# lonewolf-jp/ConvoPeq

Hardware: AMD Instinct MI355X
Metric: Mega stereo-samples/s convolved (131072-tap IR, blk=512) (higher is better)
Workload: dtype f64; 1 GPU; 256 stereo streams per GPU x 1 GPU(s) = 256 streams, 131072-tap IR (private IR per channel), blk 512, fp64 overlap-save conv + 20-band SVF EQ (bench preset, sat 0.2) [BASELINE.json configs[1]]; streams_per_gpu=256, ir_taps=131072, block=512, blocks_per_call=1024, partition=4096, eq=True, eq_preset=bench, parallelism=streams sharded rank-major, 1 rank(s), one per GPU

## Files before the change

### convopeq_amd/csrc/mac_kernels.hip

```cpp
#include "kernels.hpp"

namespace cpq {

namespace {

template <int TT, int PF, int NT = 0>
__global__ __launch_bounds__(256, (TT >= 32 || (TT == 16 && PF >= 16)) ? 1 : 2) void k_fdl_mac(const double2* __restrict__ X, const double2* __restrict__ H,
                                                 const int* __restrict__ irSlot, double2* __restrict__ Y,
                                                 int nPairs, int kPad, int ringMask, int head, int T, int nTiles,
                                                 int64_t hSlotStride, int P, int segShift, int K)
{
    static_assert(TT % PF == 0, "prefetch depth must divide the tile");
    const int bid = blockIdx.x;
    const int xcd = bid & 7;
    const int q = bid >> 3;
    const int tile = q % nTiles;
    const int pair = (q / nTiles) * 8 + xcd;
    if (pair >= nPairs) return;
    const int c = pair >> segShift;
    const int bin = (pair & ((1 << segShift) - 1)) * blockDim.x + threadIdx.x;
    const int t0 = tile * TT;

    const double2* __restrict__ Xc = X + (int64_t)c * (ringMask + 1) * P + bin;
    const double2* __restrict__ Hc = H + (int64_t)irSlot[c] * hSlotStride + bin;
    const int base = head + t0;

    constexpr bool kSplitRe = TT <= 8;
    double2 acc[TT], xw[TT], xn[PF], hn[PF];
    double accq[kSplitRe ? TT : 1];
#pragma unroll
    for (int u = 0; u < TT; ++u) {
        acc[u] = make_double2(0.0, 0.0);
        if (kSplitRe) accq[u] = 0.0;
        xw[u] = Xc[(int64_t)((base + u) & ringMask) * P];
    }
#pragma unroll
    for (int r = 0; r < PF; ++r) {
        xn[r] = Xc[(int64_t)((base - r - 1) & ringMask) * P];
        hn[r] = Hc[(int64_t)r * P];
    }

    for (int k0 = 0; k0 < kPad; k0 += TT) {
#pragma unroll
        for (int r = 0; r < TT; ++r) {
            const int k = k0 + r;
            const double2 h = hn[r % PF];
            const double2 xnew = xn[r % PF];
            if (k + PF < K) {
                if (NT >= 2) {
                    const double* hp = reinterpret_cast<const double*>(Hc + (int64_t)(k + PF) * P);
                    hn[r % PF] = make_double2(__builtin_nontemporal_load(hp), __builtin_nontemporal_load(hp + 1));
                } else {
                    hn[r % PF] = Hc[(int64_t)(k + PF) * P];
                }
            }
            if (k + PF + 1 < K) {
                if (NT >= 1) {
                    const double* xp = reinterpret_cast<const double*>(Xc + (int64_t)((base - (k + PF) - 1) & ringMask) * P);
                    xn[r % PF] = make_double2(__builtin_nontemporal_load(xp), __builtin_nontemporal_load(xp + 1));
                } else {
                    xn[r % PF] = Xc[(int64_t)((base - (k + PF) - 1) & ringMask) * P];
                }
            }
            __builtin_amdgcn_sched_barrier(0);
            if (k < K)
#pragma unroll
            for (int i = 0; i < TT; ++i) {
                const double2 x = xw[(i - r + TT) % TT];
                if (kSplitRe) {
                    acc[i].x = fma(x.x, h.x, acc[i].x);
                    accq[i] = fma(x.y, h.y, accq[i]);
                } else {
                    acc[i].x = fma(x.x, h.x, fma(-x.y, h.y, acc[i].x));
                }
                acc[i].y = fma(x.x, h.y, fma(x.y, h.x, acc[i].y));
            }
            xw[TT - 1 - r] = xnew;
            __builtin_amdgcn_sched_barrier(0);
        }
    }
#pragma unroll
    for (int i = 0; i < TT; ++i)
        if (t0 + i < T) {
            double2 y = acc[i];
            if (kSplitRe) y = (bin == 0) ? make_double2(acc[i].x, accq[i]) : make_double2(acc[i].x - accq[i], acc[i].y);
            Y[((int64_t)c * T + t0 + i) * P + bin] = y;
        }
}

constexpr int kWgWaves = 8;
constexpr int kWgTile = 8;
constexpr int kWgRingBlocks = kWgWaves + 1;
static_assert(kWgWaves == kWgTile, "k_fdl_mac_wg fetches block -1 one row per wave: waves per workgroup == rows per block");

__global__ __launch_bounds__(64 * kWgWaves, 4) void k_fdl_mac_wg(const double2* __restrict__ X,
                                                                  const double2* __restrict__ H,
                                                                  const int* __restrict__ irSlot,
                                                                  double2* __restrict__ Y, int kPad, int ringMask,
                                                                  int head, int T, int nGroups, int64_t hSlotStride,
                                                                  int P, int nCols, int nWork, int K)
{
    __shared__ double2 ring[kWgRingBlocks * kWgTile * 64];
    __shared__ double2 hst[kWgTile * 64];
    const int lane = threadIdx.x & 63;
    const int w = __builtin_amdgcn_readfirstlane(threadIdx.x >> 6);
    const int perXcd = gridDim.x >> 3;
    const int logical = (blockIdx.x & 7) * perXcd + (blockIdx.x >> 3);
    if (logical >= nWork) return;
    const int grp = logical % nGroups;
    const int cg = logical / nGroups;
    const int c = cg / nCols;
    const int bin = (cg - c * nCols) * 64 + lane;
    const int base = head + grp * (kWgWaves * kWgTile);
    const int t0w = grp * (kWgWaves * kWgTile) + w * kWgTile;

    const double2* __restrict__ Xu = X + (int64_t)c * (ringMask + 1) * P;
    const double2* __restrict__ Hu = H + (int64_t)irSlot[c] * hSlotStride;
    auto slotOf = [](int b) { return ((b % kWgRingBlocks) + kWgRingBlocks) % kWgRingBlocks; };
    auto xrow = [&](int slot) { return Xu + (int64_t)(slot & ringMask) * P; };
    auto hrow = [&](int k) { return Hu + (int64_t)k * P; };

    double m1[kWgTile], m2[kWgTile], m3[kWgTile], xsum[kWgTile];
    double2 xw[kWgTile];
#pragma unroll
    for (int u = 0; u < kWgTile; ++u) {
        m1[u] = 0.0; m2[u] = 0.0; m3[u] = 0.0;
        xw[u] = xrow(base + kWgTile * w + u)[bin];
        xsum[u] = xw[u].x + xw[u].y;
    }
    if (w < kWgWaves - 1) {
#pragma unroll
        for (int u = 0; u < kWgTile; ++u) ring[(slotOf(w) * kWgTile + u) * 64 + lane] = xw[u];
    }
    {
        const double2 xs = xrow(base - kWgTile + w)[bin];
        ring[(slotOf(-1) * kWgTile + w) * 64 + lane] = xs;
    }
    hst[w * 64 + lane] = hrow(w)[bin];
    __syncthreads();

    const int nChunks = kPad / kWgTile;
    const int rem = K - (nChunks - 1) * kWgTile;
    const bool active = t0w < T;
    for (int j = 0; j < nChunks; ++j) {
        const bool lastChunk = (j == nChunks - 1), nextIsLast = (j == nChunks - 2);
        const int steps = lastChunk ? rem : kWgTile;
        double2 xs = make_double2(0.0, 0.0), hsn = make_double2(0.0, 0.0);
        if (!lastChunk && (!nextIsLast || w > kWgTile - rem)) {
            const double* xp = reinterpret_cast<const double*>(xrow(base + kWgTile * (-j - 2) + w) + bin);
            xs = make_double2(__builtin_nontemporal_load(xp), __builtin_nontemporal_load(xp + 1));
        }
        if (!lastChunk && (!nextIsLast || w < rem))
            hsn = hrow((j + 1) * kWgTile + w)[bin];
        const double2* blk = ring + slotOf(w - j - 1) * kWgTile * 64 + lane;
        if (active)
#pragma unroll
        for (int r = 0; r < kWgTile; ++r) {
            if (r < steps) {
            const double2 h = hst[r * 64 + lane];
            const double hs = h.x + h.y;
            if (r > 0) xsum[kWgTile - r] = xw[kWgTile - r].x + xw[kWgTile - r].y;
            {
                const double2 x = xw[kWgTile - 1 - r];
                m1[kWgTile - 1] = fma(x.x, h.x, m1[kWgTile - 1]);
                m2[kWgTile - 1] = fma(x.y, h.y, m2[kWgTile - 1]);
                m3[kWgTile - 1] = fma(xsum[kWgTile - 1 - r], hs, m3[kWgTile - 1]);
            }
            xw[kWgTile - 1 - r] = blk[(kWgTile - 1 - r) * 64];
            __builtin_amdgcn_sched_barrier(0);
#pragma unroll
            for (int i = 0; i < kWgTile - 1; ++i) {
                const int sl = (i - r + kWgTile) % kWgTile;
                const double2 x = xw[sl];
                m1[i] = fma(x.x, h.x, m1[i]);
                m2[i] = fma(x.y, h.y, m2[i]);
                m3[i] = fma(xsum[sl], hs, m3[i]);
            }
            __builtin_amdgcn_sched_barrier(0);
            }
        }
        if (lastChunk) break;
        ring[(slotOf(-j - 2) * kWgTile + w) * 64 + lane] = xs;
        xsum[0] = xw[0].x + xw[0].y;
        __syncthreads();
        hst[w * 64 + lane] = hsn;
        __syncthreads();
    }
#pragma unroll
    for (int i = 0; i < kWgTile; ++i)
        if (t0w + i < T) {
            const double2 y = (bin == 0) ? make_double2(m1[i], m2[i]) : make_double2(m1[i] - m2[i], (m3[i] - m1[i]) - m2[i]);
            double* yp = reinterpret_cast<double*>(Y + ((int64_t)c * T + t0w + i) * P + bin);
            __builtin_nontemporal_store(y.x, yp);
            __builtin_nontemporal_store(y.y, yp + 1);
        }
}

__global__ __launch_bounds__(256) void k_fdl_mac_dcnyq(const double2* __restrict__ XDN,
                                                       const double2* __restrict__ HDN,
                                                       const int* __restrict__ irSlot, double2* __restrict__ Y,
                                                       int nCh, int K, int ringMask, int head, int T, int hdnStride, int P)
{
    const int lane = threadIdx.x & 63;
    const int idx = blockIdx.x * (blockDim.x >> 6) + (threadIdx.x >> 6);
    if (idx >= nCh * T) return;
    const int c = idx / T;
    const int t = idx - c * T;
    const double2* __restrict__ x = XDN + (int64_t)c * (ringMask + 1);
    const double2* __restrict__ h = HDN + (int64_t)irSlot[c] * hdnStride;
    double dc = 0.0, ny = 0.0;
    for (int k = lane; k < K; k += 64) {
        const double2 xv = x[(head + t - k) & ringMask];
        const double2 hv = h[k];
        dc = fma(xv.x, hv.x, dc);
        ny = fma(xv.y, hv.y, ny);
    }
#pragma unroll
    for (int off = 32; off > 0; off >>= 1) {
        dc += __shfl_down(dc, off);
        ny += __shfl_down(ny, off);
    }
    if (lane == 0) Y[(int64_t)idx * P] = make_double2(dc, ny);
}

template <int TT, int PF>
void launch_mac_t(hipStream_t stream, const double2* X, const double2* H, const int* irSlot, double2* Y, int P,
                  int nCh, int kPad, int K, int ringSlots, int head, int T, int64_t hSlotStride, bool hPrivate = false)
{
    const int threads = P < 256 ? P : 256;
    int segShift = 0;
    while ((threads << segShift) < P) ++segShift;
    const int nPairs = nCh << segShift;
    const int nTiles = (T + TT - 1) / TT;
    const int groups = (nPairs + 7) / 8;
    const int grid = groups * nTiles * 8;
    if constexpr (TT <= 8) {
        if (nTiles == 1) {
            if (hPrivate)
                hipLaunchKernelGGL((k_fdl_mac<TT, PF, 2>), dim3(grid), dim3(threads), 0, stream, X, H, irSlot, Y, nPairs, kPad,
                                   ringSlots - 1, head, T, nTiles, hSlotStride, P, segShift, K);
            else
                hipLaunchKernelGGL((k_fdl_mac<TT, PF, 1>), dim3(grid), dim3(threads), 0, stream, X, H, irSlot, Y, nPairs, kPad,
                                   ringSlots - 1, head, T, nTiles, hSlotStride, P, segShift, K);
            return;
        }
    }
    hipLaunchKernelGGL((k_fdl_mac<TT, PF>), dim3(grid), dim3(threads), 0, stream, X, H, irSlot, Y, nPairs, kPad,
                       ringSlots - 1, head, T, nTiles, hSlotStride, P, segShift, K);
}

}

int fdl_mac_variant(int tile, int T)
{
    if (tile) return tile;
    if (T >= 48) return 0;
    if (T >= 12) return 16;
    if (T >= 6) return 8;
    return 4;
}

bool fdl_mac_needs_dcnyq(int tile, int T) { return fdl_mac_variant(tile, T) > 8; }

int fdl_mac_kpad_align(int tile, int T)
{
    const int v = fdl_mac_variant(tile, T);
    return v == 0 ? kWgTile : v;
}

void launch_fdl_mac(hipStream_t stream, int tile, const double2* X, const double2* H, const int* irSlot, double2* Y,
                    int P, int nCh, int K, int ringSlots, int head, int T, int64_t hSlotStride, bool hPrivate)
{
    const int kAlign = fdl_mac_kpad_align(tile, T);
    const int kPad = (K + kAlign - 1) / kAlign * kAlign;
    tile = fdl_mac_variant(tile, T);
    if (tile == 0) {
        const int nGroups = (T + kWgWaves * kWgTile - 1) / (kWgWaves * kWgTile);
        const int nCols = P / 64;
        const int nWork = nCh * nCols * nGroups;
        hipLaunchKernelGGL(k_fdl_mac_wg, dim3((nWork + 7) / 8 * 8), dim3(64 * kWgWaves), 0, stream, X, H,
                           irSlot, Y, kPad, ringSlots - 1, head, T, nGroups, hSlotStride, P, nCols, nWork, K);
        return;
    }
    const int pf = 4;
#define CPQ_MAC_CASE(TT_, PF_) launch_mac_t<TT_, PF_>(stream, X, H, irSlot, Y, P, nCh, kPad, K, ringSlots, head, T, hSlotStride, hPrivate)
    switch (tile) {
        case 4:  CPQ_MAC_CASE(4, 4); break;
        case 8:  if (pf >= 8) CPQ_MAC_CASE(8, 8); else CPQ_MAC_CASE(8, 4); break;
        case 32: if (pf >= 16) CPQ_MAC_CASE(32, 16); else if (pf >= 8) CPQ_MAC_CASE(32, 8); else CPQ_MAC_CASE(32, 4); break;
        default: if (pf >= 16) CPQ_MAC_CASE(16, 16); else if (pf >= 8) CPQ_MAC_CASE(16, 8); else CPQ_MAC_CASE(16, 4); break;
    }
#undef CPQ_MAC_CASE
}

void launch_fdl_mac_dcnyq(hipStream_t stream, const double2* XDN, const double2* HDN, const int* irSlot, double2* Y,
                          int P, int nCh, int K, int ringSlots, int head, int T, int hdnStride)
{
    const int total = nCh * T;
    hipLaunchKernelGGL(k_fdl_mac_dcnyq, dim3((total + 3) / 4), dim3(256), 0, stream, XDN, HDN, irSlot, Y, nCh, K,
                       ringSlots - 1, head, T, hdnStride, P);
}

}
```

Baseline: 14970 Mega stereo-samples/s.

## Double-buffer X prefetch and use buffer loads with range-clamped predication in WG MAC

The workgroup FDL MAC kernel now issues X ring rows two chunks ahead, ping-ponging between two registers via an unrolled-by-two chunk lambda. The X and H loads become raw buffer loads whose descriptor size is set to zero or one row, so the hardware's out-of-range handling returns zero instead of relying on branches. The IR slot index is also made wave-uniform. The aim is to hide global-load latency behind the FMA loop and remove divergent control flow around loads, at the cost of extra registers and a dependence on out-of-range buffer accesses returning zero.

```diff
diff --git a/convopeq_amd/csrc/mac_kernels.hip b/convopeq_amd/csrc/mac_kernels.hip
--- a/convopeq_amd/csrc/mac_kernels.hip
+++ b/convopeq_amd/csrc/mac_kernels.hip
@@ -91,6 +91,8 @@
 constexpr int kWgWaves = 8;
 constexpr int kWgTile = 8;
 constexpr int kWgRingBlocks = kWgWaves + 1;
+constexpr int kBufferRsrcWord3 = 0x00020000;
+constexpr int kAuxNt = 2;
 static_assert(kWgWaves == kWgTile, "k_fdl_mac_wg fetches block -1 one row per wave: waves per workgroup == rows per block");
 
 __global__ __launch_bounds__(64 * kWgWaves, 4) void k_fdl_mac_wg(const double2* __restrict__ X,
@@ -115,7 +117,7 @@
     const int t0w = grp * (kWgWaves * kWgTile) + w * kWgTile;
 
     const double2* __restrict__ Xu = X + (int64_t)c * (ringMask + 1) * P;
-    const double2* __restrict__ Hu = H + (int64_t)irSlot[c] * hSlotStride;
+    const double2* __restrict__ Hu = H + (int64_t)__builtin_amdgcn_readfirstlane(irSlot[c]) * hSlotStride;
     auto slotOf = [](int b) { return ((b % kWgRingBlocks) + kWgRingBlocks) % kWgRingBlocks; };
     auto xrow = [&](int slot) { return Xu + (int64_t)(slot & ringMask) * P; };
     auto hrow = [&](int k) { return Hu + (int64_t)k * P; };
@@ -137,21 +139,36 @@
         ring[(slotOf(-1) * kWgTile + w) * 64 + lane] = xs;
     }
     hst[w * 64 + lane] = hrow(w)[bin];
-    __syncthreads();
 
     const int nChunks = kPad / kWgTile;
     const int rem = K - (nChunks - 1) * kWgTile;
     const bool active = t0w < T;
-    for (int j = 0; j < nChunks; ++j) {
+    const int col0 = (cg - c * nCols) * 64;
+    constexpr int kRowBytes = 64 * 16;
+    const int xLastRow = __builtin_amdgcn_readfirstlane(w > kWgTile - rem ? kRowBytes : 0);
+    const int hLastRow = __builtin_amdgcn_readfirstlane(w < rem ? kRowBytes : 0);
+    auto loadRow = [&]<int kAux>(const double2* row, int bytes) {
+        const uint64_t a = reinterpret_cast<uint64_t>(row + col0);
+        const uint64_t ua = ((uint64_t)(uint32_t)__builtin_amdgcn_readfirstlane((int)(a >> 32)) << 32) |
+                            (uint32_t)__builtin_amdgcn_readfirstlane((int)a);
+        const __amdgpu_buffer_rsrc_t rs = __builtin_amdgcn_make_buffer_rsrc(reinterpret_cast<void*>(ua), (short)0,
+                                                                            __builtin_amdgcn_readfirstlane(bytes),
+                                                                            kBufferRsrcWord3);
+        return __builtin_bit_cast(double2, __builtin_amdgcn_raw_buffer_load_b128(rs, lane * 16, 0, kAux));
+    };
+    auto loadX = [&](int jj) {
+        return loadRow.template operator()<kAuxNt>(xrow(base + kWgTile * (-jj - 2) + w),
+                                                   jj >= nChunks - 1 ? 0 : jj == nChunks - 2 ? xLastRow : kRowBytes);
+    };
+    double2 xsA = loadX(0), xsB;
+    __syncthreads();
+
+    auto chunk = [&](const int j, double2& xs, double2& xsNext) __attribute__((always_inline)) {
         const bool lastChunk = (j == nChunks - 1), nextIsLast = (j == nChunks - 2);
         const int steps = lastChunk ? rem : kWgTile;
-        double2 xs = make_double2(0.0, 0.0), hsn = make_double2(0.0, 0.0);
-        if (!lastChunk && (!nextIsLast || w > kWgTile - rem)) {
-            const double* xp = reinterpret_cast<const double*>(xrow(base + kWgTile * (-j - 2) + w) + bin);
-            xs = make_double2(__builtin_nontemporal_load(xp), __builtin_nontemporal_load(xp + 1));
-        }
-        if (!lastChunk && (!nextIsLast || w < rem))
-            hsn = hrow((j + 1) * kWgTile + w)[bin];
+        const double2 hsn = loadRow.template operator()<0>(hrow((j + 1) * kWgTile + w),
+                                                           lastChunk ? 0 : nextIsLast ? hLastRow : kRowBytes);
+        xsNext = loadX(j + 1);
         const double2* blk = ring + slotOf(w - j - 1) * kWgTile * 64 + lane;
         if (active)
 #pragma unroll
@@ -179,12 +196,17 @@
             __builtin_amdgcn_sched_barrier(0);
             }
         }
-        if (lastChunk) break;
+        if (lastChunk) return true;
         ring[(slotOf(-j - 2) * kWgTile + w) * 64 + lane] = xs;
         xsum[0] = xw[0].x + xw[0].y;
         __syncthreads();
         hst[w * 64 + lane] = hsn;
         __syncthreads();
+        return false;
+    };
+    for (int j = 0;; j += 2) {
+        if (chunk(j, xsA, xsB)) break;
+        if (chunk(j + 1, xsB, xsA)) break;
     }
 #pragma unroll
     for (int i = 0; i < kWgTile; ++i)
```

New measurement: 15100 Mega stereo-samples/s (median of 6 runs). About the same (+0.9%).
